# vaibhawvipul/taper

Measured on AMD Instinct MI355X. Metric: MNIST samples/sec fwd+bwd+step, higher is better.
Workload: dtype f32; 1 GPU; mlp_784-128-10_b64; per_gpu_batch=64, global_batch=64, parallelism=single, comm=none, graph_record_steps=11577

## Files before the change

include/taper_hip_debug.h:

```cpp
#ifndef TAPER_HIP_DEBUG_H
#define TAPER_HIP_DEBUG_H

#include "taper_hip.h"

#ifdef __cplusplus
extern "C" {
#endif

int th_debug_mlp3_calls(int64_t *out);
int th_debug_mlp2_calls(int64_t *out);
int th_debug_mlp2_only(int which);
int th_debug_mlp2_ksplit(int ksplit);
int th_debug_set_chain_loop(int on);
int th_debug_chain_mlp3_only(int which);
int th_debug_set_chain_generic(int on);
int th_debug_last_conv_config(th_ctx *ctx, int *out6);
int th_debug_set_conv_img(th_ctx *ctx, int mode);
int th_debug_qlinear_plan(int qtype, int batch, int in_features, int out_features, int x_misalign_bytes, int w_misalign_bytes, int *out8);
int th_debug_q8q8_plan(int batch, int in_features, int out_features, int *out4);

int th_comm_debug_dump(th_comm *comm, th_ctx *ctx);
#ifdef __cplusplus
}
#endif

#endif
```

taper_amd/csrc/adam_dev.h:

```cpp
#pragma once
#include "common.h"

namespace th {

__device__ __forceinline__ float powi_f32(float a, int b) {
    const bool recip = b < 0;
    float r = 1.0f;
    while (true) {
        if (b & 1) r *= a;
        b /= 2;
        if (b == 0) break;
        a *= a;
    }
    return recip ? 1.0f / r : r;
}

__device__ __forceinline__ float adam_step_size(float lr, float beta1, float beta2, int t) {
    const float bc1 = 1.0f - powi_f32(beta1, t);
    const float bc2 = 1.0f - powi_f32(beta2, t);
    return lr * (sqrtf(bc2) / bc1);
}

__device__ __forceinline__ void adam_update(float *__restrict__ p, float *__restrict__ m, float *__restrict__ v, long i, float grad,
                                            float step, float beta1, float beta2, float eps, float wd) {
    const float pv = p[i];
    const float gv = grad + wd * pv;
    const float mv = beta1 * m[i] + (1.0f - beta1) * gv;
    const float vv = beta2 * v[i] + (1.0f - beta2) * gv * gv;
    m[i] = mv;
    v[i] = vv;
    p[i] = pv - step * mv / (sqrtf(vv) + eps);
}

struct AdamDev {
    float *p, *m, *v;
    const int32_t *t;
    const float *lr;
    float beta1, beta2, eps, wd;
};

template <class T>
__device__ __forceinline__ T sload(const T *p) {
    return *reinterpret_cast<const __attribute__((address_space(4))) T *>(reinterpret_cast<uintptr_t>(p));
}

__device__ __forceinline__ float adam_dev_step(const AdamDev &a) { return adam_step_size(sload(a.lr), a.beta1, a.beta2, sload(a.t)); }

static inline AdamDev make_adam_dev(const th_adam_fuse *f) {
    if (!f || !f->d_p) return AdamDev{nullptr, nullptr, nullptr, nullptr, nullptr, 0.f, 0.f, 0.f, 0.f};
    return AdamDev{f->d_p, f->d_m, f->d_v, f->d_t, f->d_lr, f->beta1, f->beta2, f->eps, f->weight_decay};
}

struct AdamSlices {
    AdamDev a[TH_MAX_ADAM_SLICES];
    const float *g[TH_MAX_ADAM_SLICES];
    int64_t n[TH_MAX_ADAM_SLICES];
    int first_block[TH_MAX_ADAM_SLICES + 1];
    int count;
    const uint32_t *guard;
    uint32_t *step_word;
    int blocks() const { return first_block[count]; }
};

static inline AdamSlices make_adam_slices(const th_adam_slice *s, int n, const th_ctx *ctx) {
    AdamSlices r{};
    r.count = 0;
    r.guard = ctx ? ctx->update_guard : nullptr;
    r.step_word = ctx ? ctx->update_step_word : nullptr;
    for (int i = 0; i < n; ++i) {
        if (!s[i].f.d_p || s[i].n <= 0) continue;
        r.a[r.count] = make_adam_dev(&s[i].f);
        r.g[r.count] = s[i].d_g;
        r.n[r.count] = s[i].n;
        r.first_block[r.count + 1] = r.first_block[r.count] + (int)((s[i].n + 1023) / 1024);
        ++r.count;
    }
    for (int i = r.count; i < TH_MAX_ADAM_SLICES; ++i) r.first_block[i + 1] = r.first_block[r.count];
    return r;
}

__device__ __forceinline__ void adam_slice_quad(const AdamDev &a, const float *__restrict__ g, int64_t n, int64_t i0, float step) {
    if (i0 >= n) return;
    const bool vec = i0 + 4 <= n && ((((uintptr_t)a.p | (uintptr_t)a.m | (uintptr_t)a.v | (uintptr_t)g) & 15) == 0);
    float gv[4], pv[4], mv[4], vv[4];
    const int cnt = (int)(n - i0 < 4 ? n - i0 : 4);
    if (vec) {
        const float4 g4 = *reinterpret_cast<const float4 *>(g + i0), p4 = *reinterpret_cast<const float4 *>(a.p + i0);
        const float4 m4 = *reinterpret_cast<const float4 *>(a.m + i0), v4 = *reinterpret_cast<const float4 *>(a.v + i0);
        gv[0] = g4.x; gv[1] = g4.y; gv[2] = g4.z; gv[3] = g4.w;
        pv[0] = p4.x; pv[1] = p4.y; pv[2] = p4.z; pv[3] = p4.w;
        mv[0] = m4.x; mv[1] = m4.y; mv[2] = m4.z; mv[3] = m4.w;
        vv[0] = v4.x; vv[1] = v4.y; vv[2] = v4.z; vv[3] = v4.w;
    } else {
#pragma unroll
        for (int j = 0; j < 4; ++j) {
            const int64_t i = i0 + (j < cnt ? j : 0);
            gv[j] = g[i]; pv[j] = a.p[i]; mv[j] = a.m[i]; vv[j] = a.v[i];
        }
    }
#pragma unroll
    for (int j = 0; j < 4; ++j) {
        const float gj = gv[j] + a.wd * pv[j];
        mv[j] = a.beta1 * mv[j] + (1.0f - a.beta1) * gj;
        vv[j] = a.beta2 * vv[j] + (1.0f - a.beta2) * gj * gj;
        pv[j] = pv[j] - step * mv[j] / (sqrtf(vv[j]) + a.eps);
    }
    if (vec) {
        *reinterpret_cast<float4 *>(a.p + i0) = make_float4(pv[0], pv[1], pv[2], pv[3]);
        *reinterpret_cast<float4 *>(a.m + i0) = make_float4(mv[0], mv[1], mv[2], mv[3]);
        *reinterpret_cast<float4 *>(a.v + i0) = make_float4(vv[0], vv[1], vv[2], vv[3]);
    } else {
        for (int j = 0; j < cnt; ++j) {
            a.p[i0 + j] = pv[j]; a.m[i0 + j] = mv[j]; a.v[i0 + j] = vv[j];
        }
    }
}

__device__ __forceinline__ void adam_slices_block(const AdamSlices &x, int b) {
    if (x.guard && sload(x.guard) != 0u) return;
    int s = 0;
#pragma unroll
    for (int i = 1; i < TH_MAX_ADAM_SLICES; ++i)
        if (i < x.count && b >= x.first_block[i]) s = i;
    const AdamDev &a = x.a[s];
    const int64_t i0 = (int64_t)(b - x.first_block[s]) * 1024 + threadIdx.x * 4;
    if (i0 >= x.n[s]) return;
    adam_slice_quad(a, x.g[s], x.n[s], i0, adam_dev_step(a));
}

__device__ __forceinline__ void adam_slices_then_tick(const AdamSlices &x, int32_t *tick) {
    if (x.guard && sload(x.guard) != 0u) return;
#pragma unroll
    for (int s = 0; s < TH_MAX_ADAM_SLICES; ++s) {
        if (s >= x.count) break;
        const float step = adam_dev_step(x.a[s]);
        for (int64_t i0 = (int64_t)threadIdx.x * 4; i0 < x.n[s]; i0 += (int64_t)blockDim.x * 4) adam_slice_quad(x.a[s], x.g[s], x.n[s], i0, step);
    }
    __syncthreads();
    if (tick && threadIdx.x == 0) {
        tick[0] += 1;
        if (x.step_word) x.step_word[0] += 1u;
    }
}

}
```

taper_amd/csrc/gemm.hip:

```cpp
#include "adam_dev.h"

namespace th {

typedef float floatx4 __attribute__((ext_vector_type(4)));
typedef float floatx16 __attribute__((ext_vector_type(16)));

struct Epilogue {
    float alpha, beta;
    const float *bias;
    int relu;
    AdamDev adam;
    const float *mask;
    float *colpart;
};

static inline Epilogue make_ep(float alpha, float beta, const float *bias = nullptr, int relu = 0) {
    return Epilogue{alpha, beta, bias, relu, AdamDev{nullptr, nullptr, nullptr, nullptr, nullptr, 0.f, 0.f, 0.f, 0.f}, nullptr, nullptr};
}

__device__ __forceinline__ float epilogue_apply(float acc, float c_old, const Epilogue &ep, int col) {
    float v = ep.alpha * acc;
    if (ep.beta != 0.0f) v += ep.beta * c_old;
    if (ep.bias) v += ep.bias[col];
    if (ep.relu) v = v > 0.0f ? v : 0.0f;
    return v;
}

struct SmallArgs {
    const float *A, *Amask, *B;
    float *C, *partial;
    int m, n, k;
    long a_rs, a_cs, b_rs, b_cs;
    int kslice, a_vec, b_vec;
    Epilogue ep;
    int xcd_blocks = 0;
};

template <bool A_KC, bool B_KC, int NW, bool MASKED>
__device__ __forceinline__ void small16_body(const SmallArgs &p, int tile_row, int tile_col, int zslice, float (*red)[64][4]) {
    const int lane = threadIdx.x & 63, wave = threadIdx.x >> 6;
    const int r = lane & 15, g = lane >> 4;
    const int row0 = tile_row * 16, col0 = tile_col * 16;
    const int kbeg_slice = zslice * p.kslice;
    const int kend_slice = min(p.k, kbeg_slice + p.kslice);
    const int kwave = ((kend_slice - kbeg_slice + 16 * NW - 1) / (16 * NW)) * 16;
    const int kbeg = kbeg_slice + wave * kwave;
    const int kend = min(kend_slice, kbeg + kwave);

    const int arow = row0 + r, bcol = col0 + r;
    const bool a_ok = arow < p.m, b_ok = bcol < p.n;
    const long a_off = (long)(a_ok ? arow : 0) * p.a_rs;
    const float *ap = p.A + a_off;
    const float *mp = MASKED ? p.Amask + a_off : nullptr;
    const float *bp = p.B + (long)(b_ok ? bcol : 0) * p.b_cs;

    const int ecol = col0 + (lane & 15);
    const bool fuse_adam = p.ep.adam.p != nullptr && p.partial == nullptr;
    const int erow = row0 + (lane >> 4) * 4 + wave;
    const bool e_ok = wave < 4 && erow < p.m && ecol < p.n;
    const long e_ix = e_ok ? (long)erow * p.n + ecol : 0;
    float e_bias = 0.f, e_cold = 0.f, e_p = 0.f, e_m = 0.f, e_v = 0.f, e_step = 0.f;
    if (e_ok) {
        if (p.ep.beta != 0.0f && !p.partial) e_cold = p.C[e_ix];
        if (fuse_adam) {
            e_p = p.ep.adam.p[e_ix];
            e_m = p.ep.adam.m[e_ix];
            e_v = p.ep.adam.v[e_ix];
            e_step = adam_dev_step(p.ep.adam);
        }
        if (p.ep.bias) e_bias = p.ep.bias[ecol];
    }
    constexpr int CH = 4;
    floatx4 acc = {0.f, 0.f, 0.f, 0.f};
    for (int kk0 = kbeg; kk0 < kend; kk0 += 16 * CH) {
        float av[CH][4], bv[CH][4];
#pragma unroll
        for (int c = 0; c < CH; ++c) {
            const int kb = kk0 + 16 * c + g * 4;
            if (A_KC && p.a_vec && kb + 4 <= kend) {
                float4 t = *reinterpret_cast<const float4 *>(ap + kb);
                av[c][0] = t.x; av[c][1] = t.y; av[c][2] = t.z; av[c][3] = t.w;
                if (MASKED) {
                    float4 q = *reinterpret_cast<const float4 *>(mp + kb);
                    av[c][0] = q.x > 0.f ? av[c][0] : 0.f; av[c][1] = q.y > 0.f ? av[c][1] : 0.f;
                    av[c][2] = q.z > 0.f ? av[c][2] : 0.f; av[c][3] = q.w > 0.f ? av[c][3] : 0.f;
                }
            } else {
#pragma unroll
                for (int s = 0; s < 4; ++s) {
                    const bool in = kb + s < kend;
                    float v = in ? ap[(long)(kb + s) * p.a_cs] : 0.f;
                    if (MASKED) v = (in && mp[(long)(kb + s) * p.a_cs] > 0.f) ? v : 0.f;
                    av[c][s] = v;
                }
            }
            if (B_KC && p.b_vec && kb + 4 <= kend) {
                float4 t = *reinterpret_cast<const float4 *>(bp + kb);
                bv[c][0] = t.x; bv[c][1] = t.y; bv[c][2] = t.z; bv[c][3] = t.w;
            } else {
#pragma unroll
                for (int s = 0; s < 4; ++s) bv[c][s] = (kb + s < kend) ? bp[(long)(kb + s) * p.b_rs] : 0.f;
            }
        }
#pragma unroll
        for (int c = 0; c < CH; ++c) {
            if (kk0 + 16 * c >= kend) break;
#pragma unroll
            for (int s = 0; s < 4; ++s) {
                const float a = a_ok ? av[c][s] : 0.f;
                const float b = b_ok ? bv[c][s] : 0.f;
                acc = __builtin_amdgcn_mfma_f32_16x16x4f32(a, b, acc, 0, 0, 0);
            }
        }
    }

#pragma unroll
    for (int i = 0; i < 4; ++i) red[wave][lane][i] = acc[i];
    __syncthreads();
    if (wave < 4) {
        float sum = red[0][lane][wave];
        for (int w = 1; w < NW; ++w) sum += red[w][lane][wave];
        if (e_ok) {
            if (p.partial) {
                p.partial[(long)zslice * p.m * p.n + e_ix] = sum;
            } else {
                float out = p.ep.alpha * sum;
                if (p.ep.beta != 0.0f) out += p.ep.beta * e_cold;
                if (p.ep.bias) out += e_bias;
                if (p.ep.relu) out = out > 0.0f ? out : 0.0f;
                p.C[e_ix] = out;
                if (fuse_adam) {
                    const AdamDev &ad = p.ep.adam;
                    const float gv = out + ad.wd * e_p;
                    const float mn = ad.beta1 * e_m + (1.0f - ad.beta1) * gv;
                    const float vn = ad.beta2 * e_v + (1.0f - ad.beta2) * gv * gv;
                    ad.m[e_ix] = mn;
                    ad.v[e_ix] = vn;
                    ad.p[e_ix] = e_p - e_step * mn / (sqrtf(vn) + ad.eps);
                }
            }
        }
    }
}

template <bool A_KC, bool B_KC, int NW>
__global__ __launch_bounds__(64 * NW) void sgemm_small16(SmallArgs p) {
    __shared__ float red[NW][64][4];
    small16_body<A_KC, B_KC, NW, false>(p, blockIdx.y, blockIdx.x, blockIdx.z, red);
}

template <bool A_KC, bool B_KC, int NW>
__global__ __launch_bounds__(64 * NW) void sgemm_small16_tick(SmallArgs p, AdamSlices x, int32_t *tick) {
    __shared__ float red[NW][64][4];
    if (blockIdx.y + 1 < gridDim.y) {
        int tm = blockIdx.y, tn = blockIdx.x;
        if (p.xcd_blocks) {
            const int b = blockIdx.x + gridDim.x * blockIdx.y, q = b & 7, j = b >> 3;
            tm = 2 * (q >> 2) + (j >> 1);
            tn = 2 * (q & 3) + (j & 1);
        }
        small16_body<A_KC, B_KC, NW, false>(p, tm, tn, 0, red);
        return;
    }
    if (blockIdx.x == 0) adam_slices_then_tick(x, tick);
}

__global__ __launch_bounds__(256) void splitk_reduce4(const float *__restrict__ partial, float *__restrict__ C, long mn, int n, int kz, Epilogue ep) {
    const long i = ((long)blockIdx.x * blockDim.x + threadIdx.x) * 4;
    if (i >= mn) return;
    const bool fuse = ep.adam.p != nullptr;
    float4 pv = {0.f, 0.f, 0.f, 0.f}, mv = pv, vv = pv, c_old = pv;
    float step = 0.f;
    if (fuse) {
        pv = *reinterpret_cast<const float4 *>(ep.adam.p + i);
        mv = *reinterpret_cast<const float4 *>(ep.adam.m + i);
        vv = *reinterpret_cast<const float4 *>(ep.adam.v + i);
        step = adam_dev_step(ep.adam);
    }
    if (ep.beta != 0.0f) c_old = *reinterpret_cast<const float4 *>(C + i);
    float s[4] = {0.f, 0.f, 0.f, 0.f};
    constexpr int U = 8;
    int z = 0;
    for (; z + U <= kz; z += U) {
        float4 v[U];
#pragma unroll
        for (int u = 0; u < U; ++u) v[u] = *reinterpret_cast<const float4 *>(partial + (long)(z + u) * mn + i);
#pragma unroll
        for (int u = 0; u < U; ++u) {
            s[0] += v[u].x; s[1] += v[u].y; s[2] += v[u].z; s[3] += v[u].w;
        }
    }
    for (; z < kz; ++z) {
        const float4 v = *reinterpret_cast<const float4 *>(partial + (long)z * mn + i);
        s[0] += v.x; s[1] += v.y; s[2] += v.z; s[3] += v.w;
    }
    const float co[4] = {c_old.x, c_old.y, c_old.z, c_old.w};
    float out[4];
#pragma unroll
    for (int e = 0; e < 4; ++e) out[e] = epilogue_apply(s[e], co[e], ep, (int)((i + e) % n));
    *reinterpret_cast<float4 *>(C + i) = make_float4(out[0], out[1], out[2], out[3]);
    if (fuse) {
        const AdamDev &ad = ep.adam;
        const float p4[4] = {pv.x, pv.y, pv.z, pv.w}, m4[4] = {mv.x, mv.y, mv.z, mv.w}, v4[4] = {vv.x, vv.y, vv.z, vv.w};
        float pn[4], mo[4], vo[4];
#pragma unroll
        for (int e = 0; e < 4; ++e) {
            const float gv = out[e] + ad.wd * p4[e];
            mo[e] = ad.beta1 * m4[e] + (1.0f - ad.beta1) * gv;
            vo[e] = ad.beta2 * v4[e] + (1.0f - ad.beta2) * gv * gv;
            pn[e] = p4[e] - step * mo[e] / (sqrtf(vo[e]) + ad.eps);
        }
        *reinterpret_cast<float4 *>(ad.m + i) = make_float4(mo[0], mo[1], mo[2], mo[3]);
        *reinterpret_cast<float4 *>(ad.v + i) = make_float4(vo[0], vo[1], vo[2], vo[3]);
        *reinterpret_cast<float4 *>(ad.p + i) = make_float4(pn[0], pn[1], pn[2], pn[3]);
    }
}

__global__ __launch_bounds__(256) void splitk_reduce(const float *__restrict__ partial, float *__restrict__ C,
                                                     long mn, int n, int kz, Epilogue ep) {
    const long i = (long)blockIdx.x * blockDim.x + threadIdx.x;
    if (i >= mn) return;
    const bool fuse = ep.adam.p != nullptr;
    float pv = 0.f, mv = 0.f, vv = 0.f, step = 0.f;
    if (fuse) {
        pv = ep.adam.p[i];
        mv = ep.adam.m[i];
        vv = ep.adam.v[i];
        step = adam_dev_step(ep.adam);
    }
    const float c_old = ep.beta != 0.0f ? C[i] : 0.0f;
    float s = 0.f;
    for (int z = 0; z < kz; ++z) s += partial[(long)z * mn + i];
    const float out = epilogue_apply(s, c_old, ep, (int)(i % n));
    C[i] = out;
    if (fuse) {
        const AdamDev &ad = ep.adam;
        const float gv = out + ad.wd * pv;
        const float mn_ = ad.beta1 * mv + (1.0f - ad.beta1) * gv;
        const float vn = ad.beta2 * vv + (1.0f - ad.beta2) * gv * gv;
        ad.m[i] = mn_;
        ad.v[i] = vn;
        ad.p[i] = pv - step * mn_ / (sqrtf(vn) + ad.eps);
    }
}

static inline bool aligned16p(const void *p) { return ((uintptr_t)p & 15) == 0; }
static inline void launch_splitk_reduce(hipStream_t stream, const float *partial, float *C, long mn, int n, int kz, const Epilogue &ep) {
// ... 685 lines not shown

int gemm_dispatch(th_ctx *ctx, int trans_a, int trans_b, int m, int n, int k, const float *A, const float *B, float *C,
                  const Epilogue &ep) {
    if (m == 0 || n == 0) return 0;
    const long a_rs = trans_a ? 1 : k, a_cs = trans_a ? m : 1;
    const long b_rs = trans_b ? 1 : n, b_cs = trans_b ? k : 1;
    const bool a_kc = !trans_a, b_kc = trans_b != 0;
    const TileClass tc = gemm_tile_class(m, n, k);
#define TH_GEMM_CASE(AK, BKC)                                                                         \
    if (a_kc == AK && b_kc == BKC)                                                                          \
        return tc == TileClass::Tile64  ? launch_tile<64, AK, BKC>(ctx, A, B, C, m, n, k, a_rs, a_cs, b_rs, b_cs, ep) \
             : tc == TileClass::Tile128 ? launch_tile128<AK, BKC>(ctx, A, B, C, m, n, k, a_rs, a_cs, b_rs, b_cs, ep)  \
                                        : launch_small<AK, BKC>(ctx, A, B, C, m, n, k, a_rs, a_cs, b_rs, b_cs, ep);
    TH_GEMM_CASE(true, true)
    TH_GEMM_CASE(true, false)
    TH_GEMM_CASE(false, true)
    TH_GEMM_CASE(false, false)
#undef TH_GEMM_CASE
    return 3;
}

int mlp3_grads_launch(th_ctx *ctx, const float *const dz[3], const float *const act[3], float *const dw[3], float *const db[3],
                      const int out_f[3], const int in_f[3], const th_adam_fuse *const wf[3], const th_adam_fuse *const bf[3], int batch,
                      const float *part, int n_blk, float *loss, float *ncorrect, float *metrics, int64_t capacity, int64_t *state,
                      int64_t advance, const float *gap_dx, const th_mlp3_gap *gap) {
    Mlp3GradArgs a{};
    int blocks = 0;
    for (int l = 0; l < 3; ++l) {
        LinearBwdArgs &q = a.job[l];
        const int tm = ceil_div(out_f[l], 16), tn = ceil_div(in_f[l], 16);
        q.dw_kz = 1;
        q.dw_tiles = dw[l] ? tm * tn : 0;
        q.n_dw = (q.dw_tiles + 7) & ~7;
        q.dw_tiles_m = tm;
        q.dw = SmallArgs{dz[l], nullptr, act[l], dw[l], nullptr, out_f[l], in_f[l], batch, 1, out_f[l], in_f[l], 1, (batch + 15) / 16 * 16, 0, 0,
                         make_ep(1.0f, 0.0f)};
        q.dw.ep.adam = make_adam_dev(dw[l] ? wf[l] : nullptr);
        q.db_adam = make_adam_dev(db[l] ? bf[l] : nullptr);
        q.dy = dz[l];
        q.db = db[l];
        q.batch = batch;
        q.out_f = out_f[l];
        q.n_db = db[l] ? ceil_div(out_f[l], 64) : 0;
        a.first[l] = blocks;
        blocks += q.n_dw + q.n_db;
    }
    a.first[3] = blocks;
    if (gap && gap->d_cnt) {
        a.gap_dx = gap_dx; a.gap_cnt = gap->d_cnt; a.gap_db = gap->d_gb; a.gap_c = in_f[0]; a.gap_hw = gap->hw;
        a.gap_adam = make_adam_dev(gap->b_fuse);
        blocks += ceil_div(a.gap_c, 16);
    }
    a.first[4] = blocks;
    a.part = part; a.n_blk = n_blk; a.batch = batch;
    a.loss = loss; a.ncorrect = ncorrect; a.metrics = metrics; a.capacity = capacity; a.state = state; a.advance = advance;
    hipLaunchKernelGGL(mlp3_grads_kernel, dim3(blocks + 1), dim3(256), 0, ctx->stream, a);
    TH_LAUNCH_CHECK();
    return 0;
}

int linear_fwd_partials(th_ctx *ctx, const float *x, const float *w, int m, int n, int k, float **partial_out, int *kz_out) {
    const int tiles_m = ceil_div(m, 16), tiles_n = ceil_div(n, 16);
    const long tiles = (long)tiles_m * tiles_n;
    SmallArgs p{x, nullptr, w, nullptr, nullptr, m, n, k, k, 1, 1, k, 0, 0, 0, make_ep(1.0f, 0.0f)};
    p.a_vec = aligned16(x) && (k % 4 == 0);
    p.b_vec = aligned16(w) && (k % 4 == 0);
    int kz = (int)std::min<long>((256 + tiles - 1) / tiles, k / 512);
    if (kz < 1) kz = 1;
    if (kz > 8) kz = 8;
    const int kslice = (ceil_div(k, kz) + 15) / 16 * 16;
    kz = ceil_div(k, kslice);
    p.kslice = kslice;
    void *ws = nullptr;
    if (th_malloc(ctx, (size_t)kz * m * n * sizeof(float), &ws)) return 1;
    p.partial = (float *)ws;
    if (tiles < 256 && k >= 256) hipLaunchKernelGGL((sgemm_small16<true, true, 16>), dim3(tiles_n, tiles_m, kz), dim3(1024), 0, ctx->stream, p);
    else hipLaunchKernelGGL((sgemm_small16<true, true, 4>), dim3(tiles_n, tiles_m, kz), dim3(256), 0, ctx->stream, p);
    TH_LAUNCH_CHECK();
    *partial_out = p.partial;
    *kz_out = kz;
    return 0;
}

}

using namespace th;

extern "C" {

#ifdef TH_PROFILE
int th_debug_gemm_prof(th_ctx *ctx, long long *h_out4) {
    TH_HIP(hipStreamSynchronize(ctx->stream));
    TH_HIP(hipMemcpyFromSymbol(h_out4, HIP_SYMBOL(th::g_gemm_prof), 4 * sizeof(long long)));
    return 0;
}
#endif

int th_sgemm(th_ctx *ctx, int trans_a, int trans_b, int m, int n, int k, float alpha, const float *d_a,
             const float *d_b, float beta, float *d_c) {
    TH_REQUIRE(ctx, "th_sgemm: null ctx");
    TH_REQUIRE(m >= 0 && n >= 0 && k >= 0, "th_sgemm: negative dimension");
    TH_REQUIRE((m == 0 || n == 0) || (d_c && (k == 0 || (d_a && d_b))), "th_sgemm: null device pointer");
    Epilogue ep = make_ep(alpha, beta);
    return gemm_dispatch(ctx, trans_a, trans_b, m, n, k, d_a, d_b, d_c, ep);
}

int th_linear_fwd(th_ctx *ctx, const float *d_x, const float *d_w, const float *d_b, float *d_y, int batch,
                  int in_features, int out_features, int relu) {
    TH_REQUIRE(ctx && d_x && d_w && d_y, "th_linear_fwd: null argument");
    Epilogue ep = make_ep(1.0f, 0.0f, d_b, relu);
    return gemm_dispatch(ctx, 0, 1, batch, out_features, in_features, d_x, d_w, d_y, ep);
}

int th_linear_fwd_ex(th_ctx *ctx, const float *d_x, const float *d_w, const float *d_b, float *d_y, int batch, int in_features,
                     int out_features, int relu, const th_adam_slice *extra, int n_extra, int32_t *d_tick) {
    TH_REQUIRE(ctx && d_x && d_w && d_y, "th_linear_fwd_ex: null argument");
    TH_REQUIRE(n_extra >= 0 && n_extra <= TH_MAX_ADAM_SLICES && (n_extra == 0 || extra), "th_linear_fwd_ex: bad extra slices");
    for (int i = 0; i < n_extra; ++i)
        TH_REQUIRE(extra[i].f.d_p != d_w && extra[i].f.d_p != d_b, "th_linear_fwd_ex: a carried slice must not alias what this launch reads");
    const int m = batch, n = out_features, k = in_features;
    const long tiles = (long)ceil_div(m, 16) * ceil_div(n, 16);
    if (m > 0 && n > 0 && k > 0 && !gemm_is_big(m, n, k) && !(tiles < 64 && k >= 2048)) {
        SmallArgs p{d_x, nullptr, d_w, d_y, nullptr, m, n, k, k, 1, 1, k, (k + 15) / 16 * 16, 0, 0, make_ep(1.0f, 0.0f, d_b, relu)};
        p.a_vec = aligned16(d_x) && (k % 4 == 0);
        p.b_vec = aligned16(d_w) && (k % 4 == 0);
        const AdamSlices x = make_adam_slices(extra, n_extra, ctx);
        const dim3 grid(ceil_div(n, 16), ceil_div(m, 16) + 1, 1);
        p.xcd_blocks = grid.x == 8 && grid.y == 5;
        if (tiles < 256 && k >= 256) hipLaunchKernelGGL((sgemm_small16_tick<true, true, 16>), grid, dim3(1024), 0, ctx->stream, p, x, d_tick);
        else hipLaunchKernelGGL((sgemm_small16_tick<true, true, 4>), grid, dim3(256), 0, ctx->stream, p, x, d_tick);
        TH_LAUNCH_CHECK();
        return 0;
    }
    if (int rc = th_adam_slices(ctx, extra, n_extra)) return rc;
    if (d_tick)
        if (int rc = th_adam_tick(ctx, d_tick)) return rc;
    return th_linear_fwd(ctx, d_x, d_w, d_b, d_y, batch, in_features, out_features, relu);
}

}

namespace th {

constexpr int THIN_ROWS = 32;
__global__ __launch_bounds__(256) void linear_dx_thin_kernel(const float *__restrict__ dz, const float *__restrict__ w, const float *__restrict__ xmask,
                                                             float *__restrict__ dx, float *__restrict__ colpart, int batch, int in_f, int out_f,
                                                             int accumulate) {
    __shared__ float dzs[THIN_ROWS][16];
    const int t = threadIdx.x, r0 = blockIdx.y * THIN_ROWS, col = (blockIdx.x * 256 + t) * 4;
    for (int i = t; i < THIN_ROWS * 16; i += 256) {
        const int r = i >> 4, o = i & 15;
        dzs[r][o] = (r0 + r < batch && o < out_f) ? dz[(long)(r0 + r) * out_f + o] : 0.f;
    }
    float4 wv[16];
#pragma unroll
    for (int o = 0; o < 16; ++o) wv[o] = (o < out_f && col < in_f) ? *reinterpret_cast<const float4 *>(w + (long)o * in_f + col) : make_float4(0.f, 0.f, 0.f, 0.f);
    __syncthreads();
    if (col >= in_f) return;
    float4 cs = make_float4(0.f, 0.f, 0.f, 0.f);
#pragma unroll 8
    for (int r = 0; r < THIN_ROWS; ++r) {
        if (r0 + r >= batch) break;
        const long idx = (long)(r0 + r) * in_f + col;
        float4 v = accumulate ? *reinterpret_cast<const float4 *>(dx + idx) : make_float4(0.f, 0.f, 0.f, 0.f);
#pragma unroll
        for (int o = 0; o < 16; ++o) {
            const float d = dzs[r][o];
            v.x = fmaf(d, wv[o].x, v.x); v.y = fmaf(d, wv[o].y, v.y); v.z = fmaf(d, wv[o].z, v.z); v.w = fmaf(d, wv[o].w, v.w);
        }
        if (xmask) {
            const float4 m = *reinterpret_cast<const float4 *>(xmask + idx);
            v.x = m.x > 0.f ? v.x : 0.f; v.y = m.y > 0.f ? v.y : 0.f; v.z = m.z > 0.f ? v.z : 0.f; v.w = m.w > 0.f ? v.w : 0.f;
        }
        *reinterpret_cast<float4 *>(dx + idx) = v;
        cs.x += v.x; cs.y += v.y; cs.z += v.z; cs.w += v.w;
    }
    if (colpart) *reinterpret_cast<float4 *>(colpart + (long)blockIdx.y * in_f + col) = cs;
}

static int dx_epilogue_rows(int batch, int in_f, int out_f) {
    if (batch <= 0 || in_f <= 0 || out_f <= 0) return 0;
    if (out_f <= 16 && in_f % 4 == 0 && (long)batch * in_f >= (1L << 20)) return ceil_div(batch, THIN_ROWS);
    if (gemm_tile_class(batch, in_f, out_f) == TileClass::Tile128 && tile128_kz(batch, in_f, out_f) == 1) return ceil_div(batch, BM);
    return 0;
}

}

extern "C" {

int th_linear_bwd_dx_epilogue_rows(int batch, int in_features, int out_features) { return th::dx_epilogue_rows(batch, in_features, out_features); }

int th_linear_bwd_separate_products(int batch, int in_features, int out_features, int with_dx, int with_dw, int dx_epilogue) {
    const int ep_rows = (dx_epilogue && with_dx) ? th::dx_epilogue_rows(batch, in_features, out_features) : 0;
    const bool thin_dx = ep_rows > 0 && out_features <= 16;
    const bool dw_big = with_dw && gemm_is_big(out_features, in_features, batch);
    const bool dx_big = with_dx && !thin_dx && gemm_is_big(batch, in_features, out_features);
    return (!dw_big && !dx_big && batch <= 4096 && out_features <= 4096) ? 0 : 1;
}

int th_linear_bwd(th_ctx *ctx, const float *d_x, const float *d_w, const float *d_dy, const float *d_relu_y, float *d_dx,
                  float *d_dw, float *d_db, int batch, int in_features, int out_features, int accumulate_mask) {
    return th_linear_bwd_adam(ctx, d_x, d_w, d_dy, d_relu_y, d_dx, d_dw, d_db, batch, in_features, out_features, accumulate_mask,
                              nullptr, nullptr);
}

int th_linear_bwd_adam(th_ctx *ctx, const float *d_x, const float *d_w, const float *d_dy, const float *d_relu_y, float *d_dx,
                       float *d_dw, float *d_db, int batch, int in_features, int out_features, int accumulate_mask,
                       const th_adam_fuse *w_fuse, const th_adam_fuse *b_fuse) {
    return th_linear_bwd_adam_ex(ctx, d_x, d_w, d_dy, d_relu_y, d_dx, d_dw, d_db, batch, in_features, out_features, accumulate_mask,
                                 w_fuse, b_fuse, nullptr, 0);
}

int th_linear_bwd_adam_ex(th_ctx *ctx, const float *d_x, const float *d_w, const float *d_dy, const float *d_relu_y, float *d_dx,
                          float *d_dw, float *d_db, int batch, int in_features, int out_features, int accumulate_mask,
                          const th_adam_fuse *w_fuse, const th_adam_fuse *b_fuse, const th_adam_slice *extra, int n_extra) {
    return th_linear_bwd_adam_ex2(ctx, d_x, d_w, d_dy, d_relu_y, d_dx, d_dw, d_db, batch, in_features, out_features, accumulate_mask, w_fuse,
                                  b_fuse, extra, n_extra, 0, nullptr);
}

// ... 128 lines not shown
```

Measured before the change: 5.186 million samples/s.

## Add whole-tile fused forward GEMM with front-loaded Adam tick block

```diff
diff --git a/include/taper_hip_debug.h b/include/taper_hip_debug.h
--- a/include/taper_hip_debug.h
+++ b/include/taper_hip_debug.h
@@ -17,6 +17,7 @@
 int th_debug_last_conv_config(th_ctx *ctx, int *out6);
 int th_debug_set_conv_img(th_ctx *ctx, int mode);
 int th_debug_qlinear_plan(int qtype, int batch, int in_features, int out_features, int x_misalign_bytes, int w_misalign_bytes, int *out8);
+int th_debug_linear_fwd_ex_plan(int batch, int in_features, int out_features, int x_misalign_bytes, int w_misalign_bytes, int *out4);
 int th_debug_q8q8_plan(int batch, int in_features, int out_features, int *out4);
 
 int th_comm_debug_dump(th_comm *comm, th_ctx *ctx);
diff --git a/taper_amd/csrc/adam_dev.h b/taper_amd/csrc/adam_dev.h
--- a/taper_amd/csrc/adam_dev.h
+++ b/taper_amd/csrc/adam_dev.h
@@ -79,41 +79,66 @@
     return r;
 }
 
+typedef float adam_f4 __attribute__((ext_vector_type(4)));
+struct AdamQuad {
+    adam_f4 g, p, m, v;
+    int cnt;
+    bool vec;
+};
+
+__device__ __forceinline__ bool adam_slice_aligned16(const AdamDev &a, const float *g) {
+    return (((uintptr_t)a.p | (uintptr_t)a.m | (uintptr_t)a.v | (uintptr_t)g) & 15) == 0;
+}
+
+__device__ __forceinline__ void adam_quad_load(AdamQuad &q, const AdamDev &a, const float *__restrict__ g, int64_t n, int64_t i0, bool vec) {
+    q.cnt = i0 >= n ? 0 : (int)(n - i0 < 4 ? n - i0 : 4);
+    q.vec = vec;
+    if (q.cnt == 0) return;
+    if (vec) {
+        q.g = *reinterpret_cast<const adam_f4 *>(g + i0);
+        q.p = *reinterpret_cast<const adam_f4 *>(a.p + i0);
+        q.m = *reinterpret_cast<const adam_f4 *>(a.m + i0);
+        q.v = *reinterpret_cast<const adam_f4 *>(a.v + i0);
+    } else {
+#pragma unroll
+        for (int j = 0; j < 4; ++j) {
+            const int64_t i = i0 + (j < q.cnt ? j : 0);
+            q.g[j] = g[i]; q.p[j] = a.p[i]; q.m[j] = a.m[i]; q.v[j] = a.v[i];
+        }
+    }
+}
+
+__device__ __forceinline__ void adam_quad_update(AdamQuad &q, const AdamDev &a, float step) {
+#pragma unroll
+    for (int j = 0; j < 4; ++j) {
+        const float gj = q.g[j] + a.wd * q.p[j];
+        q.m[j] = a.beta1 * q.m[j] + (1.0f - a.beta1) * gj;
+        q.v[j] = a.beta2 * q.v[j] + (1.0f - a.beta2) * gj * gj;
+        q.p[j] = q.p[j] - step * q.m[j] / (sqrtf(q.v[j]) + a.eps);
+    }
+}
+
+__device__ __forceinline__ void adam_quad_store(const AdamQuad &q, const AdamDev &a, int64_t i0) {
+    if (q.cnt == 0) return;
+    if (q.vec) {
+        *reinterpret_cast<adam_f4 *>(a.p + i0) = q.p;
+        *reinterpret_cast<adam_f4 *>(a.m + i0) = q.m;
+        *reinterpret_cast<adam_f4 *>(a.v + i0) = q.v;
+    } else {
+#pragma unroll
+        for (int j = 0; j < 4; ++j) {
+            if (j >= q.cnt) break;
+            a.p[i0 + j] = q.p[j]; a.m[i0 + j] = q.m[j]; a.v[i0 + j] = q.v[j];
+        }
+    }
+}
+
 __device__ __forceinline__ void adam_slice_quad(const AdamDev &a, const float *__restrict__ g, int64_t n, int64_t i0, float step) {
     if (i0 >= n) return;
-    const bool vec = i0 + 4 <= n && ((((uintptr_t)a.p | (uintptr_t)a.m | (uintptr_t)a.v | (uintptr_t)g) & 15) == 0);
-    float gv[4], pv[4], mv[4], vv[4];
-    const int cnt = (int)(n - i0 < 4 ? n - i0 : 4);
-    if (vec) {
-        const float4 g4 = *reinterpret_cast<const float4 *>(g + i0), p4 = *reinterpret_cast<const float4 *>(a.p + i0);
-        const float4 m4 = *reinterpret_cast<const float4 *>(a.m + i0), v4 = *reinterpret_cast<const float4 *>(a.v + i0);
-        gv[0] = g4.x; gv[1] = g4.y; gv[2] = g4.z; gv[3] = g4.w;
-        pv[0] = p4.x; pv[1] = p4.y; pv[2] = p4.z; pv[3] = p4.w;
-        mv[0] = m4.x; mv[1] = m4.y; mv[2] = m4.z; mv[3] = m4.w;
-        vv[0] = v4.x; vv[1] = v4.y; vv[2] = v4.z; vv[3] = v4.w;
-    } else {
-#pragma unroll
-        for (int j = 0; j < 4; ++j) {
-            const int64_t i = i0 + (j < cnt ? j : 0);
-            gv[j] = g[i]; pv[j] = a.p[i]; mv[j] = a.m[i]; vv[j] = a.v[i];
-        }
-    }
-#pragma unroll
-    for (int j = 0; j < 4; ++j) {
-        const float gj = gv[j] + a.wd * pv[j];
-        mv[j] = a.beta1 * mv[j] + (1.0f - a.beta1) * gj;
-        vv[j] = a.beta2 * vv[j] + (1.0f - a.beta2) * gj * gj;
-        pv[j] = pv[j] - step * mv[j] / (sqrtf(vv[j]) + a.eps);
-    }
-    if (vec) {
-        *reinterpret_cast<float4 *>(a.p + i0) = make_float4(pv[0], pv[1], pv[2], pv[3]);
-        *reinterpret_cast<float4 *>(a.m + i0) = make_float4(mv[0], mv[1], mv[2], mv[3]);
-        *reinterpret_cast<float4 *>(a.v + i0) = make_float4(vv[0], vv[1], vv[2], vv[3]);
-    } else {
-        for (int j = 0; j < cnt; ++j) {
-            a.p[i0 + j] = pv[j]; a.m[i0 + j] = mv[j]; a.v[i0 + j] = vv[j];
-        }
-    }
+    AdamQuad q;
+    adam_quad_load(q, a, g, n, i0, i0 + 4 <= n && adam_slice_aligned16(a, g));
+    adam_quad_update(q, a, step);
+    adam_quad_store(q, a, i0);
 }
 
 __device__ __forceinline__ void adam_slices_block(const AdamSlices &x, int b) {
@@ -128,19 +153,78 @@
     adam_slice_quad(a, x.g[s], x.n[s], i0, adam_dev_step(a));
 }
 
-__device__ __forceinline__ void adam_slices_then_tick(const AdamSlices &x, int32_t *tick) {
-    if (x.guard && sload(x.guard) != 0u) return;
+#ifdef TH_PROFILE
+#define ADAM_TICK_STAMP(i)                                                      \
+    do {                                                                        \
+        __builtin_amdgcn_sched_barrier(0);                                      \
+        if (prof && threadIdx.x == 0) prof[i] = wall_clock64();                 \
+        __builtin_amdgcn_sched_barrier(0);                                      \
+    } while (0)
+#else
+#define ADAM_TICK_STAMP(i) do { } while (0)
+#endif
+
+template <class T>
+__device__ __forceinline__ T sload_or_any(const T *p) {
+    const T *any = reinterpret_cast<const T *>(reinterpret_cast<uintptr_t>(__builtin_amdgcn_kernarg_segment_ptr()));
+    return sload(p ? p : any);
+}
+
+__device__ __forceinline__ void adam_slices_then_tick(const AdamSlices &x, int32_t *tick, long long *prof = nullptr) {
+    ADAM_TICK_STAMP(0);
+    asm volatile("" ::"s"(x.guard), "s"(x.step_word), "s"(tick), "s"(x.count), "s"(x.a[0].t), "s"(x.a[0].lr), "s"(x.a[1].t), "s"(x.a[1].lr),
+                 "s"(x.a[2].t), "s"(x.a[2].lr), "s"(x.a[3].t), "s"(x.a[3].lr), "s"(x.n[0]), "s"(x.n[1]), "s"(x.n[2]), "s"(x.n[3]));
+    static_assert(TH_MAX_ADAM_SLICES == 4, "the argument batch above names four slices");
+    uint32_t guard_w = sload_or_any(x.guard), step_w = sload_or_any(x.step_word);
+    int32_t tick_w = sload_or_any(tick);
+    int32_t t[TH_MAX_ADAM_SLICES];
+    float lr[TH_MAX_ADAM_SLICES];
 #pragma unroll
     for (int s = 0; s < TH_MAX_ADAM_SLICES; ++s) {
-        if (s >= x.count) break;
-        const float step = adam_dev_step(x.a[s]);
-        for (int64_t i0 = (int64_t)threadIdx.x * 4; i0 < x.n[s]; i0 += (int64_t)blockDim.x * 4) adam_slice_quad(x.a[s], x.g[s], x.n[s], i0, step);
-    }
+        t[s] = sload_or_any(s < x.count ? x.a[s].t : nullptr);
+        lr[s] = sload_or_any(s < x.count ? x.a[s].lr : nullptr);
+    }
+    asm volatile(""
+                 : "+s"(guard_w), "+s"(step_w), "+s"(tick_w), "+s"(t[0]), "+s"(t[1]), "+s"(t[2]), "+s"(t[3]), "+s"(lr[0]), "+s"(lr[1]),
+                   "+s"(lr[2]), "+s"(lr[3])
+                 : "s"(x.a[0].p), "s"(x.a[0].m), "s"(x.a[0].v), "s"(x.g[0]), "s"(x.a[1].p), "s"(x.a[1].m), "s"(x.a[1].v), "s"(x.g[1]),
+                   "s"(x.a[2].p), "s"(x.a[2].m), "s"(x.a[2].v), "s"(x.g[2]), "s"(x.a[3].p), "s"(x.a[3].m), "s"(x.a[3].v), "s"(x.g[3]));
+    if (x.guard && guard_w != 0u) return;
     __syncthreads();
+    ADAM_TICK_STAMP(1);
     if (tick && threadIdx.x == 0) {
-        tick[0] += 1;
-        if (x.step_word) x.step_word[0] += 1u;
-    }
-}
-
-}
+        tick[0] = tick_w + 1;
+        if (x.step_word) x.step_word[0] = step_w + 1u;
+    }
+    const int64_t i0 = (int64_t)threadIdx.x * 4, stride = (int64_t)blockDim.x * 4;
+    AdamQuad q[TH_MAX_ADAM_SLICES];
+#pragma unroll
+    for (int s = 0; s < TH_MAX_ADAM_SLICES; ++s) {
+        q[s].cnt = 0;
+        q[s].vec = true;
+        if (s < x.count && adam_slice_aligned16(x.a[s], x.g[s]) && i0 + 4 <= x.n[s]) adam_quad_load(q[s], x.a[s], x.g[s], x.n[s], i0, true);
+    }
+    ADAM_TICK_STAMP(2);
+    float step[TH_MAX_ADAM_SLICES];
+#pragma unroll
+    for (int s = 0; s < TH_MAX_ADAM_SLICES; ++s) {
+        step[s] = 0.f;
+        if (s < x.count) {
+            step[s] = adam_step_size(lr[s], x.a[s].beta1, x.a[s].beta2, t[s]);
+            if (q[s].cnt) adam_quad_update(q[s], x.a[s], step[s]);
+        }
+    }
+#pragma unroll
+    for (int s = 0; s < TH_MAX_ADAM_SLICES; ++s)
+        if (s < x.count) adam_quad_store(q[s], x.a[s], i0);
+    ADAM_TICK_STAMP(3);
+#pragma unroll 1
+    for (int s = 0; s < x.count; ++s) {
+        const float st = s == 0 ? step[0] : s == 1 ? step[1] : s == 2 ? step[2] : step[3];
+        const bool done_first = adam_slice_aligned16(x.a[s], x.g[s]) && i0 + 4 <= x.n[s];
+        for (int64_t i = done_first ? i0 + stride : i0; i < x.n[s]; i += stride) adam_slice_quad(x.a[s], x.g[s], x.n[s], i, st);
+    }
+    ADAM_TICK_STAMP(4);
+}
+
+}
diff --git a/taper_amd/csrc/gemm.hip b/taper_amd/csrc/gemm.hip
--- a/taper_amd/csrc/gemm.hip
+++ b/taper_amd/csrc/gemm.hip
@@ -1,8 +1,7 @@
-#include "adam_dev.h"
+#include "tail_dev.h"
 
 namespace th {
 
-typedef float floatx4 __attribute__((ext_vector_type(4)));
 typedef float floatx16 __attribute__((ext_vector_type(16)));
 
 struct Epilogue {
@@ -36,8 +35,27 @@
     int xcd_blocks = 0;
 };
 
+#ifdef TH_PROFILE
+__device__ long long g_fwd_prof[2][8];
+#define FWD_STAMP(i)                                                            \
+    do {                                                                        \
+        __builtin_amdgcn_sched_barrier(0);                                      \
+        if (prof && threadIdx.x == 0) prof[i] = wall_clock64();                 \
+        __builtin_amdgcn_sched_barrier(0);                                      \
+    } while (0)
+#define FWD_STAMP_ARRIVED(i)                                                    \
+    do {                                                                        \
+        asm volatile("s_waitcnt vmcnt(0)" ::: "memory");                        \
+        FWD_STAMP(i);                                                           \
+    } while (0)
+#else
+#define FWD_STAMP(i) do { } while (0)
+#define FWD_STAMP_ARRIVED(i) do { } while (0)
+#endif
+
 template <bool A_KC, bool B_KC, int NW, bool MASKED>
-__device__ __forceinline__ void small16_body(const SmallArgs &p, int tile_row, int tile_col, int zslice, float (*red)[64][4]) {
+__device__ __forceinline__ void small16_body(const SmallArgs &p, int tile_row, int tile_col, int zslice, float (*red)[64][4],
+                                             long long *prof = nullptr) {
     const int lane = threadIdx.x & 63, wave = threadIdx.x >> 6;
     const int r = lane & 15, g = lane >> 4;
     const int row0 = tile_row * 16, col0 = tile_col * 16;
@@ -72,6 +90,7 @@
     }
     constexpr int CH = 4;
     floatx4 acc = {0.f, 0.f, 0.f, 0.f};
+    FWD_STAMP(1);
     for (int kk0 = kbeg; kk0 < kend; kk0 += 16 * CH) {
         float av[CH][4], bv[CH][4];
 #pragma unroll
@@ -102,6 +121,7 @@
                 for (int s = 0; s < 4; ++s) bv[c][s] = (kb + s < kend) ? bp[(long)(kb + s) * p.b_rs] : 0.f;
             }
         }
+        FWD_STAMP_ARRIVED(2);
 #pragma unroll
         for (int c = 0; c < CH; ++c) {
             if (kk0 + 16 * c >= kend) break;
@@ -117,6 +137,7 @@
 #pragma unroll
     for (int i = 0; i < 4; ++i) red[wave][lane][i] = acc[i];
     __syncthreads();
+    FWD_STAMP(3);
     if (wave < 4) {
         float sum = red[0][lane][wave];
         for (int w = 1; w < NW; ++w) sum += red[w][lane][wave];
@@ -141,6 +162,7 @@
             }
         }
     }
+    FWD_STAMP(4);
 }
 
 template <bool A_KC, bool B_KC, int NW>
@@ -149,20 +171,100 @@
     small16_body<A_KC, B_KC, NW, false>(p, blockIdx.y, blockIdx.x, blockIdx.z, red);
 }
 
-template <bool A_KC, bool B_KC, int NW>
-__global__ __launch_bounds__(64 * NW) void sgemm_small16_tick(SmallArgs p, AdamSlices x, int32_t *tick) {
+struct FwdTileArgs {
+    const float *x, *w, *bias;
+    float *y;
+    int m, n, k, relu;
+    int xcd_blocks;
+};
+
+__device__ __forceinline__ void fwd_tile_whole(const FwdTileArgs &p, int tile, float (*red)[64][4], long long *prof) {
+    constexpr int NW = 16, CH = 4;
+    const unsigned lane = threadIdx.x & 63, wave = __builtin_amdgcn_readfirstlane(threadIdx.x >> 6);
+    const unsigned r = lane & 15, g = lane >> 4;
+    const unsigned k = (unsigned)p.k, n = (unsigned)p.n, tiles_n = n >> 4;
+    unsigned tm, tn;
+    if (p.xcd_blocks) {
+        const unsigned q = tile & 7, j = tile >> 3;
+        tm = 2 * (q >> 2) + (j >> 1);
+        tn = 2 * (q & 3) + (j & 1);
+    } else {
+        tm = (unsigned)tile / tiles_n;
+        tn = (unsigned)tile - tm * tiles_n;
+    }
+    const unsigned kwave = ((k + 16 * NW - 1) / (16 * NW)) * 16;
+    const unsigned kbeg = wave * kwave;
+    const unsigned nch = kbeg < k ? (min(k, kbeg + kwave) - kbeg) >> 4 : 0u;
+    const unsigned a_off = ((tm * 16 + r) * k + g * 4) * 4u, b_off = ((tn * 16 + r) * k + g * 4) * 4u;
+    const unsigned ecol = tn * 16 + r;
+    const unsigned e_off = ((tm * 16 + g * 4 + wave) * n + ecol) * 4u;
+    unsigned koff[CH];
+#pragma unroll
+    for (int c = 0; c < CH; ++c) koff[c] = (unsigned)c < nch ? (kbeg + 16 * c) * 4u : 0u;
+    FWD_STAMP(1);
+    float4 av[CH], bv[CH];
+#pragma unroll
+    for (int c = 0; c < CH; ++c) {
+        av[c] = ldg4_b(p.x, a_off + koff[c]);
+        bv[c] = ldg4_b(p.w, b_off + koff[c]);
+    }
+    float e_bias = 0.f;
+    if (p.bias && wave < 4) e_bias = ldg_b(p.bias, ecol * 4u);
+    FWD_STAMP_ARRIVED(2);
+    floatx4 acc = {0.f, 0.f, 0.f, 0.f};
+#pragma unroll
+    for (int c = 0; c < CH; ++c) {
+        if ((unsigned)c >= nch) break;
+        acc = __builtin_amdgcn_mfma_f32_16x16x4f32(av[c].x, bv[c].x, acc, 0, 0, 0);
+        acc = __builtin_amdgcn_mfma_f32_16x16x4f32(av[c].y, bv[c].y, acc, 0, 0, 0);
+        acc = __builtin_amdgcn_mfma_f32_16x16x4f32(av[c].z, bv[c].z, acc, 0, 0, 0);
+        acc = __builtin_amdgcn_mfma_f32_16x16x4f32(av[c].w, bv[c].w, acc, 0, 0, 0);
+    }
+#pragma unroll
+    for (int i = 0; i < 4; ++i) red[wave][lane][i] = acc[i];
+    __syncthreads();
+    FWD_STAMP(3);
+    if (wave < 4) {
+        float sum = red[0][lane][wave];
+#pragma unroll
+        for (int w = 1; w < NW; ++w) sum += red[w][lane][wave];
+        float out = sum;
+        if (p.bias) out += e_bias;
+        if (p.relu) out = out > 0.0f ? out : 0.0f;
+        *reinterpret_cast<float *>(reinterpret_cast<char *>(p.y) + e_off) = out;
+    }
+    FWD_STAMP(4);
+}
+
+template <bool A_KC, bool B_KC, int NW, bool WHOLE = false>
+__global__ __launch_bounds__(64 * NW) void sgemm_small16_tick(std::conditional_t<WHOLE, FwdTileArgs, SmallArgs> p, AdamSlices x, int32_t *tick) {
     __shared__ float red[NW][64][4];
-    if (blockIdx.y + 1 < gridDim.y) {
-        int tm = blockIdx.y, tn = blockIdx.x;
+#ifdef TH_PROFILE
+    long long *prof = blockIdx.x <= 1 ? g_fwd_prof[blockIdx.x] : nullptr;
+#else
+    long long *prof = nullptr;
+#endif
+    if (blockIdx.x == 0) {
+        adam_slices_then_tick(x, tick, prof);
+        return;
+    }
+    const int b = blockIdx.x - 1;
+    if constexpr (WHOLE) {
+        static_assert(A_KC && B_KC && NW == 16, "the whole-tile instance is X . W^T on 16 waves");
+        asm volatile("" ::"s"(p.x), "s"(p.w), "s"(p.bias), "s"(p.y), "s"(p.m), "s"(p.n), "s"(p.k), "s"(p.relu), "s"(p.xcd_blocks));
+        FWD_STAMP(0);
+        fwd_tile_whole(p, b, red, prof);
+    } else {
+        FWD_STAMP(0);
+        const int tiles_n = (p.n + 15) >> 4;
+        int tm = b / tiles_n, tn = b - tm * tiles_n;
         if (p.xcd_blocks) {
-            const int b = blockIdx.x + gridDim.x * blockIdx.y, q = b & 7, j = b >> 3;
+            const int q = b & 7, j = b >> 3;
             tm = 2 * (q >> 2) + (j >> 1);
             tn = 2 * (q & 3) + (j & 1);
         }
-        small16_body<A_KC, B_KC, NW, false>(p, tm, tn, 0, red);
-        return;
-    }
-    if (blockIdx.x == 0) adam_slices_then_tick(x, tick);
+        small16_body<A_KC, B_KC, NW, false>(p, tm, tn, 0, red, prof);
+    }
 }
 
 __global__ __launch_bounds__(256) void splitk_reduce4(const float *__restrict__ partial, float *__restrict__ C, long mn, int n, int kz, Epilogue ep) {
@@ -1014,6 +1116,28 @@
     return 0;
 }
 
+enum { FWD_EX_FALLBACK = 0, FWD_EX_GENERIC4 = 1, FWD_EX_GENERIC16 = 2, FWD_EX_WHOLE = 3 };
+struct FwdExPlan {
+    int form;
+    int kwave;
+    int grid;
+    int xcd_blocks;
+};
+
+static FwdExPlan fwd_ex_plan(int m, int n, int k, uintptr_t x_bits, uintptr_t w_bits) {
+    FwdExPlan pl{};
+    const long tiles = (long)ceil_div(m, 16) * ceil_div(n, 16);
+    if (!(m > 0 && n > 0 && k > 0 && !gemm_is_big(m, n, k) && !(tiles < 64 && k >= 2048))) return pl;
+    const bool w16 = tiles < 256 && k >= 256;
+    const int nw = w16 ? 16 : 4;
+    const bool whole = w16 && m % 16 == 0 && n % 16 == 0 && k % 16 == 0 && k <= 1024 && (x_bits & 15) == 0 && (w_bits & 15) == 0;
+    pl.form = whole ? FWD_EX_WHOLE : w16 ? FWD_EX_GENERIC16 : FWD_EX_GENERIC4;
+    pl.kwave = ceil_div(k, 16 * nw) * 16;
+    pl.grid = (int)tiles + 1;
+    pl.xcd_blocks = ceil_div(n, 16) == 8 && ceil_div(m, 16) == 4;
+    return pl;
+}
+
 }
 
 using namespace th;
@@ -1021,6 +1145,11 @@
 extern "C" {
 
 #ifdef TH_PROFILE
+int th_debug_fwd_prof(th_ctx *ctx, long long *h_out16) {
+    TH_HIP(hipStreamSynchronize(ctx->stream));
+    TH_HIP(hipMemcpyFromSymbol(h_out16, HIP_SYMBOL(th::g_fwd_prof), 16 * sizeof(long long)));
+    return 0;
+}
 int th_debug_gemm_prof(th_ctx *ctx, long long *h_out4) {
     TH_HIP(hipStreamSynchronize(ctx->stream));
     TH_HIP(hipMemcpyFromSymbol(h_out4, HIP_SYMBOL(th::g_gemm_prof), 4 * sizeof(long long)));
@@ -1051,16 +1180,21 @@
     for (int i = 0; i < n_extra; ++i)
         TH_REQUIRE(extra[i].f.d_p != d_w && extra[i].f.d_p != d_b, "th_linear_fwd_ex: a carried slice must not alias what this launch reads");
     const int m = batch, n = out_features, k = in_features;
-    const long tiles = (long)ceil_div(m, 16) * ceil_div(n, 16);
-    if (m > 0 && n > 0 && k > 0 && !gemm_is_big(m, n, k) && !(tiles < 64 && k >= 2048)) {
+    const FwdExPlan pl = fwd_ex_plan(m, n, k, (uintptr_t)d_x, (uintptr_t)d_w);
+    const AdamSlices x = pl.form != FWD_EX_FALLBACK ? make_adam_slices(extra, n_extra, ctx) : AdamSlices{};
+    if (pl.form == FWD_EX_WHOLE) {
+        const FwdTileArgs p{d_x, d_w, d_b, d_y, m, n, k, relu, pl.xcd_blocks};
+        hipLaunchKernelGGL((sgemm_small16_tick<true, true, 16, true>), dim3(pl.grid), dim3(1024), 0, ctx->stream, p, x, d_tick);
+        TH_LAUNCH_CHECK();
+        return 0;
+    }
+    if (pl.form != FWD_EX_FALLBACK) {
         SmallArgs p{d_x, nullptr, d_w, d_y, nullptr, m, n, k, k, 1, 1, k, (k + 15) / 16 * 16, 0, 0, make_ep(1.0f, 0.0f, d_b, relu)};
         p.a_vec = aligned16(d_x) && (k % 4 == 0);
         p.b_vec = aligned16(d_w) && (k % 4 == 0);
-        const AdamSlices x = make_adam_slices(extra, n_extra, ctx);
-        const dim3 grid(ceil_div(n, 16), ceil_div(m, 16) + 1, 1);
-        p.xcd_blocks = grid.x == 8 && grid.y == 5;
-        if (tiles < 256 && k >= 256) hipLaunchKernelGGL((sgemm_small16_tick<true, true, 16>), grid, dim3(1024), 0, ctx->stream, p, x, d_tick);
-        else hipLaunchKernelGGL((sgemm_small16_tick<true, true, 4>), grid, dim3(256), 0, ctx->stream, p, x, d_tick);
+        p.xcd_blocks = pl.xcd_blocks;
+        if (pl.form == FWD_EX_GENERIC16) hipLaunchKernelGGL((sgemm_small16_tick<true, true, 16>), dim3(pl.grid), dim3(1024), 0, ctx->stream, p, x, d_tick);
+        else hipLaunchKernelGGL((sgemm_small16_tick<true, true, 4>), dim3(pl.grid), dim3(256), 0, ctx->stream, p, x, d_tick);
         TH_LAUNCH_CHECK();
         return 0;
     }
@@ -1068,6 +1202,16 @@
     if (d_tick)
         if (int rc = th_adam_tick(ctx, d_tick)) return rc;
     return th_linear_fwd(ctx, d_x, d_w, d_b, d_y, batch, in_features, out_features, relu);
+}
+
+int th_debug_linear_fwd_ex_plan(int batch, int in_features, int out_features, int x_misalign_bytes, int w_misalign_bytes, int *out4) {
+    TH_REQUIRE(out4, "th_debug_linear_fwd_ex_plan: null argument");
+    TH_REQUIRE(batch >= 0 && in_features >= 0 && out_features >= 0 && x_misalign_bytes >= 0 && w_misalign_bytes >= 0,
+               "th_debug_linear_fwd_ex_plan: bad shape B=%d K=%d N=%d", batch, in_features, out_features);
+    const FwdExPlan pl = fwd_ex_plan(batch, out_features, in_features, (uintptr_t)x_misalign_bytes, (uintptr_t)w_misalign_bytes);
+    const int out[4] = {pl.form, pl.kwave, pl.grid, pl.xcd_blocks};
+    std::copy(out, out + 4, out4);
+    return 0;
 }
 
 }
```

New measurement: 4.721 million samples/s. -9.0%, worse.
